# mayataka/robotoc

Hardware: NVIDIA H100
Metric: SQP-iterations/s (ANYmal N=40, batch=1024) at 1/2/4/8 H100 vs CPU ref (higher is better)
Workload: dtype f64

## Files before the change

robotoc_b200/csrc/rbt_api.cu:

```cuda
#include <cmath>
#include <cstdio>
#include <cstring>
#include <cstdint>
#include <cstdlib>
#include <string>
#include <utility>
#include <vector>

#include <cuda_runtime.h>
#include <dlfcn.h>

#include <algorithm>

#include "../../include/robotoc_b200.h"
#include "riccati_backward.cuh"
#include "riccati_forward.cuh"
#include "riccati_time_parallel.cuh"
#include "riccati_unconstr.cuh"
#include "stage_kernels.cuh"
#include "ustage_kernels.cuh"
#include "eval_kernels.cuh"
#include "line_search_kernels.cuh"
#include "rnea_kernels.cuh"
#include "contact_kernels.cuh"
// ... 732 lines not shown
  }
  RBT_CUDA(h, cudaSetDevice(h->device));
  return forward(h, full(h), (cudaStream_t)stream);
}

int rbt_stage_layout_get(const rbt_stage_dims* sdims, const char* field) {
  if (!sdims || !field) return -1;
  rbt_stage_layout S;
  rbt_make_stage_layout(sdims, &S);
  return rbt_stage_layout_field(&S, field);
}

int rbt_stage_setup(rbt_handle* h, const rbt_stage_dims* sd, const rbt_constraint_table* table) {
  if (!h || !sd || !table) return RBT_ERR_ARG;
  if (sd->nv != h->dims.nv || sd->nu != h->dims.nu || sd->ns_max != h->dims.ns_max || sd->n_passive != h->dims.n_passive ||
      sd->n_passive != sd->nv - sd->nu  ||
      sd->nf_max != 12 || table->n_box != sd->n_box || table->n_contacts != sd->n_contacts || sd->n_box > RBT_MAX_BOX_ROWS ||
      sd->n_contacts > RBT_MAX_CONTACTS || !(table->barrier > 0) || !(table->fraction_to_boundary > 0) ||
      !(table->fraction_to_boundary <= 1)) {
    h->err = "[rbt_stage_setup] invalid argument: stage dims / constraint table inconsistent with the handle";
    return RBT_ERR_ARG;
  }
  for (int r = 0; r < table->n_box; ++r) {
    const rbt_box_row& b = table->box[r];
    const int lim = (b.var == RBT_VAR_U) ? sd->nu : sd->nv;
    if (b.var < 0 || b.var > 3 || b.idx < 0 || b.idx >= lim || (b.sign != 1 && b.sign != -1)) {
      h->err = "[rbt_stage_setup] invalid argument: bad box row " + std::to_string(r);
      return RBT_ERR_ARG;
    }
  }
  if (3 * sd->nv + sd->nu > RBT_MAX_TARGETS) {
    h->err = "[rbt_stage_setup] invalid argument: too many limit targets";
    return RBT_ERR_ARG;
  }
  int tgt[RBT_MAX_TARGETS * 4 + RBT_MAX_BOX_ROWS] = {};
  for (int r = 0; r < table->n_box; ++r) {
    const rbt_box_row& b = table->box[r];
    int* t = tgt + 4 * ((b.var == RBT_VAR_U) ? 3 * sd->nv + b.idx : b.var * sd->nv + b.idx);
    int q = 0;
    while (q < 4 && t[q] != 0) ++q;
    if (q == 4) {
      h->err = "[rbt_stage_setup] invalid argument: more than 4 box rows on one variable";
      return RBT_ERR_ARG;
    }
    t[q] = (r + 1) * (b.sign < 0 ? -1 : 1);
    tgt[RBT_MAX_TARGETS * 4 + r] = b.var == RBT_VAR_Q ? 2 : (b.var == RBT_VAR_V ? 1 : 0);
  }
  if (h->stage_ready) {
    h->err = "[rbt_stage_setup] already set up on this handle (create a new handle for another constraint table)";
    return RBT_ERR_STATE;
  }
  if (h->n_grid > 0 && check_contacts(h, *sd, h->ctrl.data(), h->n_grid) != RBT_OK) return RBT_ERR_ARG;
  rbt_stage_layout S;
  rbt_make_stage_layout(sd, &S);
  {
    using C = rbt::CondCfg<CNV, CNU, CNS>;
    using MC = rbt::MjtjCfg<CNV, CNU>;
    const int gsz = (S.l_dgdf - S.l_dgdq) + ((15 * S.ncon + 1) & ~1);
    const int q0 = S.l_Quu - C::IN1A;
    const bool ok = S.l_Qxx - S.l_D == C::IN1A && S.l_Phix - S.l_Quu == C::IN1B && S.l_IDC - S.l_D == C::i_IDC &&
                    S.l_Qaa - S.l_D == C::i_Qaa && S.l_Qff - S.l_D == C::i_Qff && S.l_Qqf - S.l_D == C::i_Qqf &&
                    S.l_lx - q0 == C::i_lx && S.l_la - q0 == C::i_la && S.l_lf - q0 == C::i_lf && S.l_lu - q0 == C::i_lu &&
                    S.l_Fx - q0 == C::i_Fx && S.l_lup - q0 == C::i_lup && S.l_se3 - q0 == C::i_se3 && S.l_dgdq - S.l_ha == C::IN2 &&
                    S.l_hf - S.l_ha == C::j_hf && S.l_hx - S.l_ha == C::j_hx && S.l_hu - S.l_ha == C::j_hu &&
                    S.l_fx - S.l_ha == C::j_fx && S.l_sc - S.l_ha == C::j_sc &&
                    5 * S.ncp + gsz <= C::NVF * C::NX &&
                    S.l_J - S.l_M == MC::o_J && S.l_D - S.l_M == MC::MJ;
    if (!ok) {
      h->err = "[rbt_stage_setup] invalid argument: stage layout not supported by the compiled condensing kernel";
      return RBT_ERR_ARG;
    }
  }
  if (S.ncp > 160 || S.l_stride - S.l_dgdq > 512) {
    h->err = "[rbt_stage_setup] invalid argument: more than 160 inequality rows or more than 4 friction cones";
    return RBT_ERR_ARG;
  }
  RBT_CUDA(h, cudaSetDevice(h->device));
  const size_t per = size_t(h->batch) * h->n_grid_max, B = h->batch;
  DevBuf<double> lin, con, ex, sol, xd, steps, ones, stage_perf, perf, x0in;
  DevBuf<int> d_tgt;
  RBT_CUDA(h, zeroed(lin, per * S.l_stride));
  RBT_CUDA(h, zeroed(con, per * S.c_stride));
  RBT_CUDA(h, zeroed(ex, per * S.e_stride));
  RBT_CUDA(h, zeroed(sol, per * S.s_stride));
  RBT_CUDA(h, zeroed(xd, per * S.x_stride));
  RBT_CUDA(h, steps.ensure(B * 2));
  RBT_CUDA(h, ones.ensure(B * 2));
  RBT_CUDA(h, stage_perf.ensure(per * 4));
  RBT_CUDA(h, zeroed(perf, B * 8));
  RBT_CUDA(h, x0in.ensure(B * 2 * h->dims.nv));
  RBT_CUDA(h, d_tgt.ensure(sizeof(tgt) / sizeof(int)));
  RBT_CUDA(h, cudaMemcpy(d_tgt.get(), tgt, sizeof(tgt), cudaMemcpyHostToDevice));
  const std::vector<double> one(B * 2, 1.0);
  RBT_CUDA(h, cudaMemcpy(ones.get(), one.data(), one.size() * 8, cudaMemcpyHostToDevice));
  RBT_CUDA(h, cudaMemcpy(steps.get(), one.data(), one.size() * 8, cudaMemcpyHostToDevice));
  h->sdims = *sd;
  h->table = *table;
  h->S = S;
  h->d_lin.own = std::move(lin);
  h->d_con.own = std::move(con);
  h->d_ex.own = std::move(ex);
  h->d_sol.own = std::move(sol);
  h->d_xd.own = std::move(xd);
  h->d_steps = std::move(steps);
  h->d_ones = std::move(ones);
  h->d_stage_perf = std::move(stage_perf);
  h->d_perf = std::move(perf);
  h->d_x0in = std::move(x0in);
  h->d_tgt = std::move(d_tgt);
  h->stage_ready = true;
  return RBT_OK;
}

static rbt::StageParams make_stage_params(rbt_handle* h, Win w) {
  rbt::StageParams p;
  const rbt_stage_layout& S = h->S;
  const size_t g0 = w.rec();
  p.K = h->L;
  p.S = S;
  p.tab = h->table;
  p.ctrl = h->d_ctrl.get();
  p.n_grid = h->n_grid;
  p.batch = w.nb;
  p.lin = h->d_lin.get() + g0 * S.l_stride;
  p.con = h->d_con.get() + g0 * S.c_stride;
  p.kkt = h->d_kkt.get() + g0 * h->L.k_stride;
  p.ex = h->d_ex.get() + g0 * S.e_stride;
  p.dir = h->d_dir.get() + g0 * h->L.d_stride;
  p.xd = h->d_xd.get() + g0 * S.x_stride;
  p.sol = h->d_sol.get() + g0 * S.s_stride;
  p.steps = h->d_steps.get() + 2 * size_t(w.b0);
  p.info = h->d_info.get() + w.b0;
  p.tgt = reinterpret_cast<const int4*>(h->d_tgt.get());
  p.row_level = h->d_tgt.get() + RBT_MAX_TARGETS * 4;
  return p;
}

#define RBT_STAGE_CHECK(h, what)                                  \
  if (!(h)) return RBT_ERR_ARG;                                   \
  if (!(h)->stage_ready || (h)->n_grid == 0) {                    \
    (h)->err = "[" what "] stage layer not set up / no schedule"; \
    return RBT_ERR_STATE;                                         \
  }                                                               \
  RBT_CUDA(h, cudaSetDevice((h)->device));

static int condense(rbt_handle* h, Win w, cudaStream_t st) {
  using C = rbt::CondCfg<CNV, CNU, CNS>;
  auto kern = rbt::condense_kernel<CNV, CNU, CNS>;
  if (!h->attr_cond) {
    RBT_CUDA(h, cudaFuncSetAttribute(kern, cudaFuncAttributeMaxDynamicSharedMemorySize, (int)C::SMEM_BYTES));
    h->attr_cond = true;
  }
  RBT_CUDA(h, cudaMemsetAsync(h->d_info.get() + w.b0, 0, size_t(w.nb) * sizeof(int), st));
  rbt::mjtjinv_kernel<CNV, CNU><<<(w.nb * h->n_grid + 1) / 2, 64, 0, st>>>(make_stage_params(h, w));
  RBT_CUDA(h, cudaGetLastError());
  if (h->ev_condense_mid) RBT_CUDA(h, cudaEventRecord(h->ev_condense_mid, st));
  kern<<<w.nb * h->n_grid, C::NTHREADS, C::SMEM_BYTES, st>>>(make_stage_params(h, w));
  RBT_CUDA(h, cudaGetLastError());
  h->launches += 2;
  h->keep_info = true;
  h->kkt_from_condense = true;
  return RBT_OK;
}

int rbt_condense(rbt_handle* h, void* stream) {
  RBT_STAGE_CHECK(h, "rbt_condense");
  return condense(h, full(h), (cudaStream_t)stream);
}

int rbt_set_condense_event(rbt_handle* h, void* cuda_event) {
  if (!h) return RBT_ERR_ARG;
  h->ev_condense_mid = (cudaEvent_t)cuda_event;
  return RBT_OK;
}

static int expand(rbt_handle* h, Win w, cudaStream_t st) {
  RBT_CUDA(h, cudaMemcpyAsync(h->d_steps.get() + 2 * size_t(w.b0), h->d_ones.get(), size_t(w.nb) * 2 * 8, cudaMemcpyDeviceToDevice, st));
  rbt::expand_kernel<CNV, CNU, CNS><<<w.nb * h->n_grid, rbt::XTHR, 0, st>>>(make_stage_params(h, w));
  RBT_CUDA(h, cudaGetLastError());
  h->launches += 1;
  return RBT_OK;
}

int rbt_expand_and_step_sizes(rbt_handle* h, void* stream) {
  RBT_STAGE_CHECK(h, "rbt_expand_and_step_sizes");
  return expand(h, full(h), (cudaStream_t)stream);
}

static int update(rbt_handle* h, Win w, cudaStream_t st) {
  rbt::update_kernel<CNV, CNU, CNS><<<w.nb * h->n_grid, rbt::XTHR, 0, st>>>(make_stage_params(h, w));
  RBT_CUDA(h, cudaGetLastError());
  h->launches += 1;
  return RBT_OK;
}

int rbt_update(rbt_handle* h, void* stream) {
  RBT_STAGE_CHECK(h, "rbt_update");
  return update(h, full(h), (cudaStream_t)stream);
}

static rbt::EvalParams make_eval_params(rbt_handle* h, Win w) {
  rbt::EvalParams q;
  q.sp = make_stage_params(h, w);
  q.stage_perf = h->d_stage_perf.get() + w.rec() * 4;
  q.perf = h->d_perf.get() + size_t(w.b0) * 8;
  q.x0in = h->d_x0in.get() + size_t(w.b0) * 2 * h->dims.nv;
  q.dx0 = h->d_dx0.get() + size_t(w.b0) * h->L.nx;
  return q;
}

int rbt_eval_kkt(rbt_handle* h, void* stream) {
  RBT_STAGE_CHECK(h, "rbt_eval_kkt");
  cudaStream_t st = (cudaStream_t)stream;
  const rbt::EvalParams q = make_eval_params(h, full(h));
  rbt::perf_index_kernel<<<(h->batch * h->n_grid + 3) / 4, 128, 0, st>>>(q);
  rbt::perf_reduce_kernel<<<(h->batch + 127) / 128, 128, 0, st>>>(q);
  RBT_CUDA(h, cudaGetLastError());
  h->launches += 2;
  return RBT_OK;
}

int rbt_set_slack_and_dual_positive(rbt_handle* h, void* stream) {
  RBT_STAGE_CHECK(h, "rbt_set_slack_and_dual_positive");
  const rbt::EvalParams q = make_eval_params(h, full(h));
  const long long total = (long long)h->batch * h->n_grid * h->S.ncp;
  rbt::slack_dual_positive_kernel<<<unsigned((total + 255) / 256), 256, 0, (cudaStream_t)stream>>>(q);
  RBT_CUDA(h, cudaGetLastError());
  h->launches += 1;
  return RBT_OK;
}

int rbt_set_joint_limits(rbt_handle* h, const double* bound_host) {
  if (!h || !bound_host) return RBT_ERR_ARG;
  if (!h->stage_ready) {
    h->err = "[rbt_set_joint_limits] stage layer not set up";
    return RBT_ERR_STATE;
  }
  RBT_CUDA(h, cudaSetDevice(h->device));
  RBT_CUDA(h, h->d_limits.ensure(RBT_MAX_BOX_ROWS));
  RBT_CUDA(h, cudaMemcpy(h->d_limits.get(), bound_host, sizeof(double) * h->table.n_box, cudaMemcpyHostToDevice));
  return RBT_OK;
}

int rbt_linearize_joint_limits(rbt_handle* h, void* stream) {
  RBT_STAGE_CHECK(h, "rbt_linearize_joint_limits");
  if (!h->d_limits.get()) {
    h->err = "[rbt_linearize_joint_limits] call rbt_set_joint_limits first";
    return RBT_ERR_STATE;
  }
  const rbt::EvalParams q = make_eval_params(h, full(h));
  const long long total = (long long)h->batch * h->n_grid * (3 * h->S.nv + h->S.nu);
  rbt::linearize_joint_limits_kernel<<<unsigned((total + 255) / 256), 256, 0, (cudaStream_t)stream>>>(q, h->d_limits.get());
  RBT_CUDA(h, cudaGetLastError());
  h->launches += 1;
  return RBT_OK;
}

int rbt_set_robot_model(rbt_handle* h, const rbt_robot_model* m) {
  if (!h || !m) return RBT_ERR_ARG;
  if (!h->stage_ready) {
    h->err = "[rbt_set_robot_model] stage layer not set up";
    return RBT_ERR_STATE;
  }
  auto bad = [&](const std::string& what) {
    h->err = "[rbt_set_robot_model] invalid argument: " + what;
    return RBT_ERR_ARG;
  };
  if (m->nv != h->S.nv || m->n_bodies != m->nv - 5 || m->n_bodies > RBT_MAX_BODIES) return bad("nv / n_bodies disagree with the handle");
  if (m->n_contacts != h->S.ncon) return bad("n_contacts disagrees with the stage layer");
  rbt::RneaModel d = {};
  d.nb = m->n_bodies;
  d.ncon = m->n_contacts;
  for (int b = 0; b < m->n_bodies; ++b) {
    const std::string tag = "body " + std::to_string(b) + ": ";
    if (b == 0 ? m->parent[b] != -1 : (m->parent[b] < 0 || m->parent[b] >= b)) return bad(tag + "parent must come earlier in the order");
    if (!(m->mass[b] > 0.0)) return bad(tag + "mass must be positive");
    const double* I = m->inertia[b];
    double imax = 0.0;
    for (int e = 0; e < 9; ++e) imax = std::max(imax, std::fabs(I[e]));
    for (int i = 0; i < 3; ++i)
      for (int j = 0; j < i; ++j)
        if (!(std::fabs(I[i + 3 * j] - I[j + 3 * i]) <= 1e-12 * imax)) return bad(tag + "inertia is not symmetric");
    const double m1 = I[0], m2 = I[0] * I[4] - I[1] * I[3];
    const double m3 = I[0] * (I[4] * I[8] - I[5] * I[7]) - I[3] * (I[1] * I[8] - I[2] * I[7]) + I[6] * (I[1] * I[5] - I[2] * I[4]);
    if (!(m1 > 0.0 && m2 > 0.0 && m3 > 0.0)) return bad(tag + "inertia is not positive definite");
    if (b > 0) {
      const double* u = m->axis[b];
      if (!(std::fabs(std::sqrt(u[0] * u[0] + u[1] * u[1] + u[2] * u[2]) - 1.0) <= 1e-12)) return bad(tag + "axis is not a unit vector");
    }
    d.parent[b] = m->parent[b];
    for (int e = 0; e < 3; ++e) {
      d.axis[b][e] = m->axis[b][e];
      d.p[b][e] = m->placement[b][9 + e];
      d.com[b][e] = m->com[b][e];
    }
    for (int e = 0; e < 9; ++e) {
      d.R[b][e] = m->placement[b][e];
      d.Ic[b][e] = I[e];
    }
    d.mass[b] = m->mass[b];
  }
  for (int c = 0; c < m->n_contacts; ++c) {
    if (m->contact_parent[c] < 0 || m->contact_parent[c] >= m->n_bodies) return bad("contact " + std::to_string(c) + ": no such parent body");
    d.cparent[c] = m->contact_parent[c];
    for (int e = 0; e < 9; ++e) d.cR[c][e] = m->contact_placement[c][e];
    for (int e = 0; e < 3; ++e) d.cp[c][e] = m->contact_placement[c][9 + e];
  }
// ... 707 lines not shown
```

robotoc_b200/csrc/stage_kernels.cuh:

```cuda
#pragma once
#include "rbt_device.cuh"
#include "riccati_backward.cuh"
#include "../../include/rbt_stage_layout.h"

namespace rbt {

#define RBT_MAX_TARGETS 96
struct StageParams {
  rbt_layout K;
  rbt_stage_layout S;
  rbt_constraint_table tab;
  const rbt_stage_ctrl* ctrl;
  int n_grid;
  int batch;
  const double* lin;
  double* con;
  double* kkt;
  double* ex;
  double* dir;
  double* xd;
  double* sol;
  double* steps;
  int* info;
  const int4* tgt;
  const int* row_level;
};

__device__ __forceinline__ void cta_gemm(int ta, int tb, int m, int n, int k, double alpha, const double* A, int lda,
                                         const double* B, int ldb, double beta, double* C, int ldc) {
  for (int e = threadIdx.x; e < m * n; e += blockDim.x) {
    const int i = e % m, j = e / m;
    double acc = 0.0;
    for (int l = 0; l < k; ++l) {
      const double a = ta ? A[l + i * lda] : A[i + l * lda];
      const double b = tb ? B[j + l * ldb] : B[l + j * ldb];
      acc = fma(a, b, acc);
    }
    const double c0 = (beta == 0.0) ? 0.0 : beta * C[i + j * ldc];
    C[i + j * ldc] = fma(alpha, acc, c0);
  }
}

__device__ __forceinline__ void inv3_dev(const double* A, int lda, double* B, int ldb) {
  const double a = A[0], b = A[lda], c = A[2 * lda], d = A[1], e = A[1 + lda], f = A[1 + 2 * lda], g = A[2], h = A[2 + lda],
               i = A[2 + 2 * lda];
  const double det = a * (e * i - f * h) - b * (d * i - f * g) + c * (d * h - e * g);
  const double r = 1.0 / det;
  B[0] = (e * i - f * h) * r; B[ldb] = (c * h - b * i) * r; B[2 * ldb] = (b * f - c * e) * r;
  B[1] = (f * g - d * i) * r; B[1 + ldb] = (a * i - c * g) * r; B[1 + 2 * ldb] = (c * d - a * f) * r;
  B[2] = (d * h - e * g) * r; B[2 + ldb] = (b * g - a * h) * r; B[2 + 2 * ldb] = (a * e - b * d) * r;
}

__device__ __noinline__ void se3_jac_inverse_dev(const double* Jac, double* Jinv) {
  double tmp[9];
  for (int q = 0; q < 36; ++q) Jinv[q] = 0.0;
  inv3_dev(Jac, 6, Jinv, 6);
  inv3_dev(Jac + 3 + 18, 6, Jinv + 3 + 18, 6);
  for (int j = 0; j < 3; ++j)
    for (int i = 0; i < 3; ++i) {
      double acc = 0.0;
      for (int l = 0; l < 3; ++l) acc = fma(Jac[i + (3 + l) * 6], Jinv[(3 + l) + (3 + j) * 6], acc);
      tmp[i + 3 * j] = acc;
    }
  for (int j = 0; j < 3; ++j)
    for (int i = 0; i < 3; ++i) {
      double acc = 0.0;
      for (int l = 0; l < 3; ++l) acc = fma(Jinv[i + l * 6], tmp[l + 3 * j], acc);
      Jinv[i + (3 + j) * 6] = -acc;
    }
}

template <int NMAX, int LD>
__device__ __forceinline__ bool warp_cholesky_ld(double* A, int n, double* dinv) {
  static_assert(NMAX <= 32 && NMAX % 2 == 0 && LD % 2 == 0, "one row per lane; 16-byte column loads of row pairs");
  const int lane = threadIdx.x & 31;
  double a[NMAX];
#pragma unroll
  for (int k = 0; k < NMAX; ++k) a[k] = (lane < n) ? ((k <= lane && k < n) ? A[lane + k * LD] : 0.0) : ((k == lane) ? 1.0 : 0.0);
  bool ok = true;
#pragma unroll
  for (int j = 0; j < NMAX; ++j) {
    const double d = __shfl_sync(0xffffffffu, a[j], j);
    ok = ok && (d > 0.0);
    const double inv = fast_rsqrt(d);
    const double lij = a[j] * inv;
    if (lane >= j && lane < NMAX) A[lane + j * LD] = lij;
    if (lane == j) dinv[j] = inv;
    __syncwarp();
#pragma unroll
    for (int k0 = (j + 1) & ~1; k0 < NMAX; k0 += 2) {
      const double2 l2 = *reinterpret_cast<const double2*>(A + k0 + j * LD);
      if (k0 > j) a[k0] = fma(-lij, l2.x, a[k0]);
      a[k0 + 1] = fma(-lij, l2.y, a[k0 + 1]);
    }
  }
  __syncwarp();
  return ok;
}

template <int M, int N, int K, class FA, class FB, class ST>
__device__ __forceinline__ void warp_gemm(FA fa, FB fb, ST st) {
  constexpr int TM_ = num_tiles(M), TN_ = num_tiles(N);
  const int lane = threadIdx.x & 31, g = lane >> 2, t = lane & 3;
#pragma unroll
  for (int m = 0; m < TM_; ++m) {
    const int i0 = tile_off(m, M);
    double acc[TN_][2];
#pragma unroll
    for (int n = 0; n < TN_; ++n) acc[n][0] = acc[n][1] = 0.0;
    warp_mma_band<K, TN_, N>(acc, i0, fa, fb);
#pragma unroll
    for (int n = 0; n < TN_; ++n) {
      const int j0 = tile_off(n, N);
      st(i0 + g, j0 + 2 * t, acc[n][0]);
      st(i0 + g, j0 + 2 * t + 1, acc[n][1]);
    }
  }
}

template <int NV, int NFM>
struct MjtjCfg {
  static constexpr int WARPS = 2;
  static constexpr int o_L = 0, o_J = o_L + ((NV * NV + 1) & ~1), o_X = o_J + ((NFM * NV + 1) & ~1), o_W = o_X + NV * NV,
                       o_S = o_W + NV * NFM, o_Y = o_S + NFM * NFM, o_d = o_Y + NFM * NFM, o_bar = o_d + 32,
                       PER_WARP = o_bar + 2;
  static constexpr int MJ = o_X;
};

template <int NV, int NFM>
__global__ void __launch_bounds__(32 * MjtjCfg<NV, NFM>::WARPS, 10) mjtjinv_kernel(const StageParams p) {
  using C = MjtjCfg<NV, NFM>;
  constexpr int NVF = NV + NFM;
  __shared__ __align__(16) double smem[C::WARPS * C::PER_WARP];
  const rbt_stage_layout& S = p.S;
  const int lane = threadIdx.x & 31, wid = threadIdx.x >> 5;
  const size_t o = size_t(blockIdx.x) * C::WARPS + wid;
  if (o >= size_t(p.batch) * p.n_grid) return;
  const int i = int(o % p.n_grid), b = int(o / p.n_grid);
  const rbt_stage_ctrl c = p.ctrl[i];
  if (c.type == RBT_TERMINAL) return;
  const int nf = c.nf;
  const double* lin = p.lin + o * S.l_stride;
  double* Z = p.ex + o * S.e_stride + S.e_Z;
  double* sL = smem + wid * C::PER_WARP + C::o_L;
  double* sX = smem + wid * C::PER_WARP + C::o_X;
  double* sJ = smem + wid * C::PER_WARP + C::o_J;
  double* sW = smem + wid * C::PER_WARP + C::o_W;
  double* sS = smem + wid * C::PER_WARP + C::o_S;
  double* sY = smem + wid * C::PER_WARP + C::o_Y;
  double* dinv = smem + wid * C::PER_WARP + C::o_d;
  uint64_t* bar = reinterpret_cast<uint64_t*>(smem + wid * C::PER_WARP + C::o_bar);
  int bad = 0;
  if (lane == 0) {
    mbar_init(bar, 1);
    fence_mbar_init();
    mbar_expect_tx(bar, uint32_t(C::MJ) * 8u);
    tma_load_1d(sL, lin + S.l_M, uint32_t(C::MJ) * 8u, bar);
  }
  for (int e = lane; e < NFM * NFM; e += 32) sY[e] = 0.0;
  __syncwarp();
  mbar_wait(bar, 0);
  for (int e = lane; e < NFM * NV; e += 32)
    if ((e % NFM) >= nf) sJ[e] = 0.0;
  __syncwarp();
  if (!warp_cholesky_ld<NV, NV>(sL, NV, dinv)) bad |= 4;
  __syncwarp();
  if (lane < NV) {
    double x[NV];
#pragma unroll
    for (int a = 0; a < NV; ++a) x[a] = (a == lane) ? 1.0 : 0.0;
#pragma unroll
    for (int k = 0; k < NV; ++k) {
      x[k] *= dinv[k];
#pragma unroll
      for (int a0 = (k + 1) & ~1; a0 < NV; a0 += 2) {
        const double2 l2 = *reinterpret_cast<const double2*>(sL + a0 + k * NV);
        if (a0 > k) x[a0] = fma(-l2.x, x[k], x[a0]);
        if (a0 + 1 < NV) x[a0 + 1] = fma(-l2.y, x[k], x[a0 + 1]);
      }
    }
#pragma unroll
    for (int a = 0; a < NV; ++a) sX[a + lane * NV] = x[a];
  }
  __syncwarp();
  if (nf > 0) {
    warp_gemm<NV, NFM, NV>([&](int ii, int k) { return sX[ii + k * NV]; }, [&](int k, int j) { return sJ[j + k * NFM]; },
                           [&](int ii, int j, double v) { sW[ii + j * NV] = v; });
    __syncwarp();
    warp_gemm<NFM, NFM, NV>([&](int ii, int k) { return sW[k + ii * NV]; }, [&](int k, int j) { return sW[k + j * NV]; },
                            [&](int ii, int j, double v) { sS[ii + j * NFM] = v; });
    __syncwarp();
    if (!warp_cholesky_ld<NFM, NFM>(sS, nf, dinv)) bad |= 8;
    __syncwarp();
    if (lane < nf) {
      double x[NFM];
#pragma unroll
      for (int a = 0; a < NFM; ++a) x[a] = (a == lane) ? 1.0 : 0.0;
#pragma unroll
      for (int k = 0; k < NFM; ++k) {
        x[k] *= dinv[k];
#pragma unroll
        for (int a0 = (k + 1) & ~1; a0 < NFM; a0 += 2) {
          const double2 l2 = *reinterpret_cast<const double2*>(sS + a0 + k * NFM);
          if (a0 > k) x[a0] = fma(-l2.x, x[k], x[a0]);
          if (a0 + 1 < NFM) x[a0 + 1] = fma(-l2.y, x[k], x[a0 + 1]);
        }
      }
#pragma unroll
      for (int a = 0; a < NFM; ++a) sY[a + lane * NFM] = x[a];
    }
    __syncwarp();
    warp_gemm<NV, NFM, NFM>([&](int ii, int k) { return sW[ii + k * NV]; }, [&](int k, int j) { return sY[j + k * NFM]; },
                            [&](int ii, int j, double v) { sJ[ii + j * NV] = v; });
    __syncwarp();
    warp_gemm<NV, NFM, NV>([&](int ii, int k) { return sX[k + ii * NV]; }, [&](int k, int j) { return sJ[k + j * NV]; },
                           [&](int ii, int j, double v) { sW[ii + j * NV] = v; });
  } else {
    for (int e = lane; e < NV * NFM; e += 32) sW[e] = 0.0;
  }
  __syncwarp();
  {
    constexpr int TV_ = num_tiles(NV);
    const int g = lane >> 2, t = lane & 3;
#pragma unroll
    for (int m = 0; m < TV_; ++m) {
      const int i0 = tile_off(m, NV);
      double acc[TV_][2];
#pragma unroll
      for (int n = 0; n < TV_; ++n) acc[n][0] = acc[n][1] = 0.0;
      warp_mma_band<NV, TV_, NV>(acc, i0, [&](int ii, int k) { return sX[k + ii * NV]; },
                                 [&](int k, int j) { return sX[k + j * NV]; });
      warp_mma_band<NFM, TV_, NV>(acc, i0, [&](int ii, int l) { return -sW[ii + l * NV]; },
                                  [&](int l, int j) { return sW[j + l * NV]; });
#pragma unroll
      for (int n = 0; n < TV_; ++n) {
        const int j0 = tile_off(n, NV);
        Z[(i0 + g) + (j0 + 2 * t) * NVF] = acc[n][0];
        Z[(i0 + g) + (j0 + 2 * t + 1) * NVF] = acc[n][1];
      }
    }
  }
  warp_gemm<NV, NFM, NFM>([&](int ii, int l) { return sW[ii + l * NV]; }, [&](int l, int j) { return sY[l + j * NFM]; },
                          [&](int ii, int j, double v) {
                            Z[ii + (NV + j) * NVF] = v;
                            Z[(NV + j) + ii * NVF] = v;
                          });
  warp_gemm<NFM, NFM, NFM>([&](int ii, int k) { return -sY[k + ii * NFM]; }, [&](int k, int j) { return sY[k + j * NFM]; },
                           [&](int ii, int j, double v) { Z[(NV + ii) + (NV + j) * NVF] = v; });
  bad = __reduce_or_sync(0xffffffffu, bad);
  if (lane == 0 && bad) atomicOr(&p.info[b], bad);
}

template <int NV, int NU, int NFM>
struct CondCfg {
  static constexpr int NX = 2 * NV, NVF = NV + NFM;
  static constexpr int TX = num_tiles(NX), TF = num_tiles(NVF), TV = num_tiles(NV), TU = num_tiles(NU), TM = num_tiles(NFM);
  static constexpr int NWARPS = TX;
  static constexpr int NTHREADS = 32 * NWARPS;
  static constexpr int up2(int x) { return (x + 1) & ~1; }
  static constexpr int i_D = 0, i_IDC = i_D + up2(NVF * NX), i_Qaa = i_IDC + up2(NVF), i_Qff = i_Qaa + up2(NV),
                       i_Qqf = i_Qff + up2(NFM * NFM), IN1A = i_Qqf + up2(NV * NFM);
  static constexpr int i_Quu = IN1A, i_lx = i_Quu + up2(NU * NU), i_la = i_lx + up2(NX), i_lf = i_la + up2(NV),
                       i_lu = i_lf + up2(NFM), i_Fx = i_lu + up2(NU), i_lup = i_Fx + up2(NX), i_se3 = i_lup + 6,
                       IN1 = i_se3 + 108, IN1B = IN1 - IN1A;
  static constexpr int j_ha = 0, j_hf = j_ha + up2(NV), j_hx = j_hf + up2(NFM), j_hu = j_hx + up2(NX), j_fx = j_hu + up2(NU),
                       j_sc = j_fx + up2(NX), IN2 = j_sc + 4;
  static constexpr int o_in1 = 0;
  static constexpr int o_Z = o_in1 + IN1;
  static constexpr int o_R = o_Z + NVF * NVF;
  static constexpr int o_in2 = o_R + NVF * NX;
  static constexpr int o_vec = o_in2 + IN2;
  static constexpr int v_r = 0, v_laf = NVF, v_haf = 2 * NVF, v_Fi = 3 * NVF, v_FiS = v_Fi + 36, v_dQq = v_FiS + 36,
                       v_dQv = v_dQq + NV * NV, v_end = v_dQv + up2(NV);
  static constexpr int o_bar = (o_vec + v_end + 1) & ~1;
  static constexpr int SMEM_DOUBLES = o_bar + 2;
  static constexpr size_t SMEM_BYTES = size_t(SMEM_DOUBLES) * 8;
  static constexpr int QAF = 0, QUF = NFM * NX;
  static_assert(TF < NWARPS && TV <= NWARPS && 2 * TM < NWARPS, "one warp per row band, one warp left for the vectors");
  static_assert(NFM * NX + NFM * NV <= NVF * NX, "Qaf | Quf fit in the dIDCdqv buffer");
  static_assert((NFM * NX) % 2 == 0 && (NFM * NV) % 2 == 0, "Qaf | Quf are adjacent in the expansion record (one bulk store)");
};

#ifndef RBT_COND_MIN_CTAS
#define RBT_COND_MIN_CTAS 5
#endif
template <int NV, int NU, int NFM>
__global__ void __launch_bounds__(CondCfg<NV, NU, NFM>::NTHREADS, RBT_COND_MIN_CTAS) condense_kernel(const StageParams p) {
  using C = CondCfg<NV, NU, NFM>;
  constexpr int NX = C::NX, NVF = C::NVF, NTHR = C::NTHREADS, TX = C::TX, TF = C::TF, TV = C::TV, TU = C::TU, TM = C::TM;
  extern __shared__ __align__(16) double smem[];
  const rbt_layout& K = p.K;
  const rbt_stage_layout& S = p.S;
  const int tid = threadIdx.x, warp = tid >> 5, lane = tid & 31, g = lane >> 2, t = lane & 3;
  const size_t o = blockIdx.x;
  if (o >= size_t(p.batch) * p.n_grid) return;
  const int i = int(o % p.n_grid);
  const rbt_stage_ctrl c = p.ctrl[i];
  const double* lin = p.lin + o * S.l_stride;
  double* con = p.con + o * S.c_stride;
  double* kkt = p.kkt + o * K.k_stride;
  double* ex = p.ex + o * S.e_stride;
  constexpr int np = NV - NU;

  if (c.type == RBT_TERMINAL) {
    for (int e = tid; e < NX * NX; e += NTHR) kkt[K.k_Qxx + e] = lin[S.l_Qxx + e];
    for (int e = tid; e < NX; e += NTHR) kkt[K.k_lx + e] = lin[S.l_lx + e];
    if (np == 6 && tid == 0) se3_jac_inverse_dev(lin + S.l_se3 + 36, ex + S.e_Fqqpi);
    return;
  }
  const bool impact = (c.type == RBT_IMPACT);
  const bool pdipm = !impact || p.tab.impact_friction_cone != 0;
  const int nf = c.nf, nvf = NV + nf, ns = impact ? 0 : c.ns;
  const double dt = c.dt;
  double* in1 = smem + C::o_in1;
  double* sD = in1 + C::i_D;
  double* sQaf = sD + C::QAF;
  double* sQuf = sD + C::QUF;
  double* vIDC = in1 + C::i_IDC;
  double* vQaa = in1 + C::i_Qaa;
  double* sQff = in1 + C::i_Qff;
  double* sQqf = in1 + C::i_Qqf;
  const double* gQxx = lin + S.l_Qxx;
  double* gQuu = in1 + C::i_Quu;
  double* vlx = in1 + C::i_lx;
  double* vla = in1 + C::i_la;
  double* vlf = in1 + C::i_lf;
  double* vlu = in1 + C::i_lu;
  double* vFx = in1 + C::i_Fx;
  const double* vlup = in1 + C::i_lup;
  const double* sse3 = in1 + C::i_se3;
  double* sZ = smem + C::o_Z;
  double* sR = smem + C::o_R;
  const double* in2 = smem + C::o_in2;
  const double* vha = in2 + C::j_ha;
  const double* vhf = in2 + C::j_hf;
  const double* vhx = in2 + C::j_hx;
  const double* vhu = in2 + C::j_hu;
  const double* vfx = in2 + C::j_fx;
  const double* vsc = in2 + C::j_sc;
  double* vec = smem + C::o_vec;
  double* vr = vec + C::v_r;
  double* vlaf = vec + C::v_laf;
  double* vhaf = vec + C::v_haf;
  double* Fi = vec + C::v_Fi;
  double* FiS = vec + C::v_FiS;
  double* dQq = vec + C::v_dQq;
  double* dQv = vec + C::v_dQv;
  uint64_t* bar = reinterpret_cast<uint64_t*>(smem + C::o_bar);
  const int ncp = S.ncp, nbox = p.tab.n_box, ncon = p.tab.n_contacts, nc = S.nc;
  double* cSl = sR;
  double* sDq = sR + 3 * ncp;
  double* sDf = sDq + (S.l_dgdf - S.l_dgdq);
  const int gsz = (S.l_dgdf - S.l_dgdq) + ((15 * ncon + 1) & ~1);
  double* cW = sDq + ((gsz + 1) & ~1);
  double* cC = cW + ncp;

  if (tid == 0) {
    mbar_init(bar, 1);
    fence_mbar_init();
    uint32_t bytes = uint32_t(C::IN1 + NVF * NVF + C::IN2) * 8u;
    if (pdipm) bytes += uint32_t(3 * ncp + gsz) * 8u;
    mbar_expect_tx(bar, bytes);
    l2_prefetch_bulk(lin + S.l_Qxx, uint32_t(NX * NX) * 8u);
    tma_load_1d(in1, lin + S.l_D, uint32_t(C::IN1A) * 8u, bar);
    tma_load_1d(in1 + C::IN1A, lin + S.l_Quu, uint32_t(C::IN1B) * 8u, bar);
    tma_load_1d(sZ, ex + S.e_Z, uint32_t(NVF * NVF) * 8u, bar);
    tma_load_1d(smem + C::o_in2, lin + S.l_ha, uint32_t(C::IN2) * 8u, bar);
    if (pdipm) {
      tma_load_1d(cSl, con + S.c_slack, uint32_t(3 * ncp) * 8u, bar);
      tma_load_1d(sDq, lin + S.l_dgdq, uint32_t(gsz) * 8u, bar);
    }
  }
  __syncthreads();
  if (np == 6) {
    if (tid == 32 || tid == 33)
      se3_jac_inverse_dev(lin + S.l_se3 + (tid == 32 ? 36 : 72), tid == 32 ? ex + S.e_Fqqpi : Fi);
  }
  mbar_wait(bar, 0);

  if (nf < NFM) {
    for (int e = tid; e < NFM * NFM; e += NTHR)
      if ((e % NFM) >= nf || (e / NFM) >= nf) sQff[e] = 0.0;
    for (int e = nf * NV + tid; e < NV * NFM; e += NTHR) sQqf[e] = 0.0;
  }
  if (tid < NVF) {
    if (tid >= nvf) vIDC[tid] = 0.0;
    vhaf[tid] = impact ? 0.0 : (tid < NV ? vha[tid] : (tid - NV < nf ? -vhf[tid - NV] : 0.0));
    if (tid >= NV && tid - NV >= nf) vlf[tid - NV] = 0.0;
  }
  for (int e = tid; e < NV * NV + NV; e += NTHR) dQq[e] = 0.0;
  if (pdipm) {
    const double mu = p.tab.barrier;
    for (int r = tid; r < nc; r += NTHR) {
      const bool cone = r >= nbox;
      if (!cone && (impact || __ldg(p.row_level + r) + c.ineq_gate > 2)) {
        cW[r] = 0.0;
        cC[r] = 0.0;
        continue;
      }
      const bool act = !cone || ((c.contact_mask >> ((r - nbox) / 5)) & 1);
      double w = 0.0, cd = 0.0;
      if (act) {
        const double sl = cSl[r], du = cSl[ncp + r];
// ... 782 lines not shown
```

Baseline: 211,000.

## Replace blockwise Cholesky KKT inverse with register-resident Gauss-Jordan inversion per warp

The mass-matrix/contact-Jacobian KKT inverse was computed via two Cholesky factorizations, triangular inverses, a Schur complement and several tensor-core GEMMs staged through shared memory. It is now a single in-register Gauss-Jordan elimination on the full symmetric indefinite KKT matrix, with each lane holding a 4x8 block and pivot rows and columns broadcast through small shared buffers. One warp per block with a register cap replaces two warps per block, and the launch math now follows the configured warp count. This removes many shared-memory round trips and syncs, but pivots without row exchange on an indefinite matrix, which may be less numerically robust, and the register cap may cause spills.

```diff
diff --git a/robotoc_b200/csrc/rbt_api.cu b/robotoc_b200/csrc/rbt_api.cu
--- a/robotoc_b200/csrc/rbt_api.cu
+++ b/robotoc_b200/csrc/rbt_api.cu
@@ -908,7 +908,8 @@
     h->attr_cond = true;
   }
   RBT_CUDA(h, cudaMemsetAsync(h->d_info.get() + w.b0, 0, size_t(w.nb) * sizeof(int), st));
-  rbt::mjtjinv_kernel<CNV, CNU><<<(w.nb * h->n_grid + 1) / 2, 64, 0, st>>>(make_stage_params(h, w));
+  constexpr int KW = rbt::MjtjCfg<CNV, CNU>::WARPS;
+  rbt::mjtjinv_kernel<CNV, CNU><<<(w.nb * h->n_grid + KW - 1) / KW, 32 * KW, 0, st>>>(make_stage_params(h, w));
   RBT_CUDA(h, cudaGetLastError());
   if (h->ev_condense_mid) RBT_CUDA(h, cudaEventRecord(h->ev_condense_mid, st));
   kern<<<w.nb * h->n_grid, C::NTHREADS, C::SMEM_BYTES, st>>>(make_stage_params(h, w));
diff --git a/robotoc_b200/csrc/stage_kernels.cuh b/robotoc_b200/csrc/stage_kernels.cuh
--- a/robotoc_b200/csrc/stage_kernels.cuh
+++ b/robotoc_b200/csrc/stage_kernels.cuh
@@ -70,185 +70,109 @@
     }
 }
 
-template <int NMAX, int LD>
-__device__ __forceinline__ bool warp_cholesky_ld(double* A, int n, double* dinv) {
-  static_assert(NMAX <= 32 && NMAX % 2 == 0 && LD % 2 == 0, "one row per lane; 16-byte column loads of row pairs");
-  const int lane = threadIdx.x & 31;
-  double a[NMAX];
-#pragma unroll
-  for (int k = 0; k < NMAX; ++k) a[k] = (lane < n) ? ((k <= lane && k < n) ? A[lane + k * LD] : 0.0) : ((k == lane) ? 1.0 : 0.0);
-  bool ok = true;
-#pragma unroll
-  for (int j = 0; j < NMAX; ++j) {
-    const double d = __shfl_sync(0xffffffffu, a[j], j);
-    ok = ok && (d > 0.0);
-    const double inv = fast_rsqrt(d);
-    const double lij = a[j] * inv;
-    if (lane >= j && lane < NMAX) A[lane + j * LD] = lij;
-    if (lane == j) dinv[j] = inv;
-    __syncwarp();
-#pragma unroll
-    for (int k0 = (j + 1) & ~1; k0 < NMAX; k0 += 2) {
-      const double2 l2 = *reinterpret_cast<const double2*>(A + k0 + j * LD);
-      if (k0 > j) a[k0] = fma(-lij, l2.x, a[k0]);
-      a[k0 + 1] = fma(-lij, l2.y, a[k0 + 1]);
-    }
-  }
-  __syncwarp();
-  return ok;
-}
-
-template <int M, int N, int K, class FA, class FB, class ST>
-__device__ __forceinline__ void warp_gemm(FA fa, FB fb, ST st) {
-  constexpr int TM_ = num_tiles(M), TN_ = num_tiles(N);
-  const int lane = threadIdx.x & 31, g = lane >> 2, t = lane & 3;
-#pragma unroll
-  for (int m = 0; m < TM_; ++m) {
-    const int i0 = tile_off(m, M);
-    double acc[TN_][2];
-#pragma unroll
-    for (int n = 0; n < TN_; ++n) acc[n][0] = acc[n][1] = 0.0;
-    warp_mma_band<K, TN_, N>(acc, i0, fa, fb);
-#pragma unroll
-    for (int n = 0; n < TN_; ++n) {
-      const int j0 = tile_off(n, N);
-      st(i0 + g, j0 + 2 * t, acc[n][0]);
-      st(i0 + g, j0 + 2 * t + 1, acc[n][1]);
-    }
-  }
-}
-
 template <int NV, int NFM>
 struct MjtjCfg {
-  static constexpr int WARPS = 2;
-  static constexpr int o_L = 0, o_J = o_L + ((NV * NV + 1) & ~1), o_X = o_J + ((NFM * NV + 1) & ~1), o_W = o_X + NV * NV,
-                       o_S = o_W + NV * NFM, o_Y = o_S + NFM * NFM, o_d = o_Y + NFM * NFM, o_bar = o_d + 32,
-                       PER_WARP = o_bar + 2;
-  static constexpr int MJ = o_X;
+  static constexpr int WARPS = 1, REGS = 88;
+  static constexpr int o_J = (NV * NV + 1) & ~1, MJ = o_J + ((NFM * NV + 1) & ~1);
+  static constexpr int o_row = 0, o_col = 64, o_rcp = 128;
+  static constexpr int o_bar = MJ, PER_WARP = o_bar + 2;
+  static_assert(o_rcp + 32 <= MJ, "the pivot buffers reuse the staging area");
 };
 
 template <int NV, int NFM>
-__global__ void __launch_bounds__(32 * MjtjCfg<NV, NFM>::WARPS, 10) mjtjinv_kernel(const StageParams p) {
+__global__ void __launch_bounds__(32 * MjtjCfg<NV, NFM>::WARPS) __maxnreg__((MjtjCfg<NV, NFM>::REGS)) mjtjinv_kernel(const StageParams p) {
   using C = MjtjCfg<NV, NFM>;
   constexpr int NVF = NV + NFM;
+  static_assert(NVF <= 32, "A is held as 8 x 4 blocks of 4 x 8");
   __shared__ __align__(16) double smem[C::WARPS * C::PER_WARP];
   const rbt_stage_layout& S = p.S;
   const int lane = threadIdx.x & 31, wid = threadIdx.x >> 5;
-  const size_t o = size_t(blockIdx.x) * C::WARPS + wid;
-  if (o >= size_t(p.batch) * p.n_grid) return;
-  const int i = int(o % p.n_grid), b = int(o / p.n_grid);
-  const rbt_stage_ctrl c = p.ctrl[i];
+  const int o = blockIdx.x * C::WARPS + wid;
+  if (o >= p.batch * p.n_grid) return;
+  const rbt_stage_ctrl c = p.ctrl[o % p.n_grid];
   if (c.type == RBT_TERMINAL) return;
-  const int nf = c.nf;
-  const double* lin = p.lin + o * S.l_stride;
-  double* Z = p.ex + o * S.e_stride + S.e_Z;
-  double* sL = smem + wid * C::PER_WARP + C::o_L;
-  double* sX = smem + wid * C::PER_WARP + C::o_X;
-  double* sJ = smem + wid * C::PER_WARP + C::o_J;
-  double* sW = smem + wid * C::PER_WARP + C::o_W;
-  double* sS = smem + wid * C::PER_WARP + C::o_S;
-  double* sY = smem + wid * C::PER_WARP + C::o_Y;
-  double* dinv = smem + wid * C::PER_WARP + C::o_d;
-  uint64_t* bar = reinterpret_cast<uint64_t*>(smem + wid * C::PER_WARP + C::o_bar);
-  int bad = 0;
+  const int nf = c.nf, n = NV + nf;
+  const double* lin = p.lin + size_t(o) * S.l_stride;
+  double* sw = smem + wid * C::PER_WARP;
+  uint64_t* bar = reinterpret_cast<uint64_t*>(sw + C::o_bar);
   if (lane == 0) {
     mbar_init(bar, 1);
     fence_mbar_init();
     mbar_expect_tx(bar, uint32_t(C::MJ) * 8u);
-    tma_load_1d(sL, lin + S.l_M, uint32_t(C::MJ) * 8u, bar);
-  }
-  for (int e = lane; e < NFM * NFM; e += 32) sY[e] = 0.0;
+    tma_load_1d(sw, lin + S.l_M, uint32_t(C::MJ) * 8u, bar);
+  }
   __syncwarp();
   mbar_wait(bar, 0);
-  for (int e = lane; e < NFM * NV; e += 32)
-    if ((e % NFM) >= nf) sJ[e] = 0.0;
+  const int rg = lane & 7, cg = lane >> 3;
+  double a[4][8];
+#pragma unroll
+  for (int s = 0; s < 4; ++s)
+#pragma unroll
+    for (int t = 0; t < 8; ++t) {
+      const int r = rg + 8 * s, q = 8 * cg + t;
+      double v = 0.0;
+      if (r < n && q < n) {
+        if (r < NV && q < NV) v = sw[max(r, q) + min(r, q) * NV];
+        else if (r < NV) v = sw[C::o_J + (q - NV) + r * NFM];
+        else if (q < NV) v = sw[C::o_J + (r - NV) + q * NFM];
+      }
+      a[s][t] = v;
+    }
   __syncwarp();
-  if (!warp_cholesky_ld<NV, NV>(sL, NV, dinv)) bad |= 4;
-  __syncwarp();
-  if (lane < NV) {
-    double x[NV];
-#pragma unroll
-    for (int a = 0; a < NV; ++a) x[a] = (a == lane) ? 1.0 : 0.0;
-#pragma unroll
-    for (int k = 0; k < NV; ++k) {
-      x[k] *= dinv[k];
-#pragma unroll
-      for (int a0 = (k + 1) & ~1; a0 < NV; a0 += 2) {
-        const double2 l2 = *reinterpret_cast<const double2*>(sL + a0 + k * NV);
-        if (a0 > k) x[a0] = fma(-l2.x, x[k], x[a0]);
-        if (a0 + 1 < NV) x[a0 + 1] = fma(-l2.y, x[k], x[a0 + 1]);
-      }
-    }
-#pragma unroll
-    for (int a = 0; a < NV; ++a) sX[a + lane * NV] = x[a];
-  }
-  __syncwarp();
-  if (nf > 0) {
-    warp_gemm<NV, NFM, NV>([&](int ii, int k) { return sX[ii + k * NV]; }, [&](int k, int j) { return sJ[j + k * NFM]; },
-                           [&](int ii, int j, double v) { sW[ii + j * NV] = v; });
+  double* rcp = sw + C::o_rcp;
+  int bad = 0;
+#pragma unroll
+  for (int k = 0; k < NVF; ++k) {
+    if (k >= n) break;
+    const int ks = k >> 3, kr = k & 7;
+    double* prow = sw + C::o_row + (k & 1) * 32;
+    double* pcol = sw + C::o_col + (k & 1) * 32;
+    if (rg == kr) {
+#pragma unroll
+      for (int t0 = 0; t0 < 8; t0 += 2)
+        *reinterpret_cast<double2*>(prow + 8 * cg + t0) = make_double2(a[ks][t0], a[ks][t0 + 1]);
+    }
+    if (cg == ks) {
+#pragma unroll
+      for (int s = 0; s < 4; ++s) pcol[rg + 8 * s] = a[s][kr];
+      if (rg == kr) {
+        const double d = a[ks][kr];
+        if (k < NV ? !(d > 0.0) : !(d < 0.0)) bad |= (k < NV) ? 4 : 8;
+        rcp[k] = fast_rcp(d);
+      }
+    }
     __syncwarp();
-    warp_gemm<NFM, NFM, NV>([&](int ii, int k) { return sW[k + ii * NV]; }, [&](int k, int j) { return sW[k + j * NV]; },
-                            [&](int ii, int j, double v) { sS[ii + j * NFM] = v; });
-    __syncwarp();
-    if (!warp_cholesky_ld<NFM, NFM>(sS, nf, dinv)) bad |= 8;
-    __syncwarp();
-    if (lane < nf) {
-      double x[NFM];
-#pragma unroll
-      for (int a = 0; a < NFM; ++a) x[a] = (a == lane) ? 1.0 : 0.0;
-#pragma unroll
-      for (int k = 0; k < NFM; ++k) {
-        x[k] *= dinv[k];
-#pragma unroll
-        for (int a0 = (k + 1) & ~1; a0 < NFM; a0 += 2) {
-          const double2 l2 = *reinterpret_cast<const double2*>(sS + a0 + k * NFM);
-          if (a0 > k) x[a0] = fma(-l2.x, x[k], x[a0]);
-          if (a0 + 1 < NFM) x[a0 + 1] = fma(-l2.y, x[k], x[a0 + 1]);
-        }
-      }
-#pragma unroll
-      for (int a = 0; a < NFM; ++a) sY[a + lane * NFM] = x[a];
-    }
-    __syncwarp();
-    warp_gemm<NV, NFM, NFM>([&](int ii, int k) { return sW[ii + k * NV]; }, [&](int k, int j) { return sY[j + k * NFM]; },
-                            [&](int ii, int j, double v) { sJ[ii + j * NV] = v; });
-    __syncwarp();
-    warp_gemm<NV, NFM, NV>([&](int ii, int k) { return sX[k + ii * NV]; }, [&](int k, int j) { return sJ[k + j * NV]; },
-                           [&](int ii, int j, double v) { sW[ii + j * NV] = v; });
-  } else {
-    for (int e = lane; e < NV * NFM; e += 32) sW[e] = 0.0;
-  }
-  __syncwarp();
-  {
-    constexpr int TV_ = num_tiles(NV);
-    const int g = lane >> 2, t = lane & 3;
-#pragma unroll
-    for (int m = 0; m < TV_; ++m) {
-      const int i0 = tile_off(m, NV);
-      double acc[TV_][2];
-#pragma unroll
-      for (int n = 0; n < TV_; ++n) acc[n][0] = acc[n][1] = 0.0;
-      warp_mma_band<NV, TV_, NV>(acc, i0, [&](int ii, int k) { return sX[k + ii * NV]; },
-                                 [&](int k, int j) { return sX[k + j * NV]; });
-      warp_mma_band<NFM, TV_, NV>(acc, i0, [&](int ii, int l) { return -sW[ii + l * NV]; },
-                                  [&](int l, int j) { return sW[j + l * NV]; });
-#pragma unroll
-      for (int n = 0; n < TV_; ++n) {
-        const int j0 = tile_off(n, NV);
-        Z[(i0 + g) + (j0 + 2 * t) * NVF] = acc[n][0];
-        Z[(i0 + g) + (j0 + 2 * t + 1) * NVF] = acc[n][1];
-      }
-    }
-  }
-  warp_gemm<NV, NFM, NFM>([&](int ii, int l) { return sW[ii + l * NV]; }, [&](int l, int j) { return sY[l + j * NFM]; },
-                          [&](int ii, int j, double v) {
-                            Z[ii + (NV + j) * NVF] = v;
-                            Z[(NV + j) + ii * NVF] = v;
-                          });
-  warp_gemm<NFM, NFM, NFM>([&](int ii, int k) { return -sY[k + ii * NFM]; }, [&](int k, int j) { return sY[k + j * NFM]; },
-                           [&](int ii, int j, double v) { Z[(NV + ii) + (NV + j) * NVF] = v; });
+    const double rk = rcp[k];
+    double g[4];
+#pragma unroll
+    for (int s = 0; s < 4; ++s) g[s] = (s == ks && rg == kr) ? 0.0 : pcol[rg + 8 * s] * rk;
+#pragma unroll
+    for (int t0 = 0; t0 < 8; t0 += 2) {
+      const double2 r2 = *reinterpret_cast<const double2*>(prow + 8 * cg + t0);
+#pragma unroll
+      for (int s = 0; s < 4; ++s) {
+        a[s][t0] = fma(-g[s], r2.x, a[s][t0]);
+        a[s][t0 + 1] = fma(-g[s], r2.y, a[s][t0 + 1]);
+      }
+    }
+    if (cg == ks) {
+#pragma unroll
+      for (int s = 0; s < 4; ++s) a[s][kr] = (s == ks && rg == kr) ? 1.0 : -g[s];
+    }
+  }
+  double* Z = p.ex + size_t(o) * S.e_stride + S.e_Z;
+#pragma unroll
+  for (int s = 0; s < 4; ++s) {
+    const int r = rg + 8 * s;
+    const double cr = (r < n) ? rcp[r] : 0.0;
+#pragma unroll
+    for (int t = 0; t < 8; ++t) {
+      const int q = 8 * cg + t;
+      if (r < NVF && q < NVF) Z[r + q * NVF] = (r < n && q < n) ? cr * a[s][t] : 0.0;
+    }
+  }
   bad = __reduce_or_sync(0xffffffffu, bad);
-  if (lane == 0 && bad) atomicOr(&p.info[b], bad);
+  if (lane == 0 && bad) atomicOr(&p.info[o / p.n_grid], bad);
 }
 
 template <int NV, int NU, int NFM>
```

Result: faster. 213,900, median of 6 (+1.4%).
